# hzykent/LiDAL

Hardware: AMD Instinct MI355X
Metric: voxels/sec SPVCNN fwd+bwd @120k pts (higher is better)
Workload: dtype bf16; 1 GPU; spvcnn train step (train.py:127-140: fwd + CE + bwd + Adam), 5 scans x ~120k pts per GPU, 0.05 m voxels, kernel maps rebuilt every step (each step builds the next step's coordinate tables on a second stream; variants.inline_geometry: built inside the forward pass); parallelism=dp1

## Files before the change

include/lidal_amd.h:

```cpp
#ifndef LIDAL_AMD_H
#define LIDAL_AMD_H

#include <stdint.h>

#ifdef __cplusplus
extern "C" {
#endif

#define LIDAL_F32 0
#define LIDAL_BF16 1
#define LIDAL_F32_SPLIT 2

const char* lidal_last_error(void);
int lidal_version(void);

int lidal_hash(const int32_t* coords, int64_t n, int64_t* out, void* stream);
int lidal_floor_coords(const float* coords, int64_t n, int stride, int32_t* out, void* stream);
int lidal_revoxelize_coords(const float* coords, int64_t n, float init_res, float after_res, float* out_float,
                            int32_t* out_floor, void* stream);
int lidal_kernel_hash(const int32_t* coords, int64_t n, const int32_t* offsets, int k,
                      int64_t* out, void* stream);

int64_t lidal_hash_table_bytes(int64_t n_keys);
int lidal_hash_table_build(const int64_t* keys, int64_t n, void* table, int64_t table_bytes,
// ... 141 lines not shown
int lidal_conv_wgrad_streams(const void* a, const void* b, int64_t n_a, int64_t n_b, const int32_t* spairs,
                             const int32_t* sdesc, int n_wg, int a_col, float* gw, float* partial, int64_t n_slabs,
                             int k, int ca, int cb, int dtype, void* stream);

int64_t lidal_bn_workspace_bytes(int64_t n, int c);
int lidal_bn_train_fwd(const void* x, int dtype, int64_t n, int c, const float* gamma,
                       const float* beta, float eps, float momentum, float* running_mean,
                       float* running_var, int64_t* num_batches_tracked, int relu,
                       const void* residual, void* y, float* save_mean, float* save_invstd, void* ws,
                       int64_t ws_bytes, void* stream);
int lidal_bn_train_fwd_tiles(const void* x, int dtype, int64_t n, int c, const float* gamma,
                             const float* beta, float eps, float momentum, float* running_mean,
                             float* running_var, int64_t* num_batches_tracked, int relu,
                             const void* residual, void* y, float* save_mean, float* save_invstd,
                             const float* tile_stats, int64_t n_tiles, void* stream);
int lidal_bn_eval_fwd(const void* x, int dtype, int64_t n, int c, const float* gamma,
                      const float* beta, const float* running_mean, const float* running_var,
                      float eps, int relu, void* y, void* stream);
int lidal_bn_bwd(const void* x, const void* dy, int64_t dy_stride, int dtype, int64_t n, int c, const float* gamma,
                 const float* beta, int relu, const float* save_mean, const float* save_invstd,
                 void* dx, float* grad_gamma, float* grad_beta, void* ws, int64_t ws_bytes,
                 void* stream);
int lidal_bn_bwd_tiles(const void* x, const void* dy, int64_t dy_stride, int dtype, int64_t n, int c,
                       const float* gamma, const float* beta, int relu, const float* save_mean,
                       const float* save_invstd, void* dx, float* grad_gamma, float* grad_beta,
                       const float* tile_sums, int64_t n_tiles, void* stream);
int lidal_add_relu_bwd_bn_sums(const void* out, const void* g, void* gm, int dtype, int64_t n, int c,
                               const void* x_a, const float* mean_a, const float* invstd_a, void* part_a,
                               const void* x_b, const float* mean_b, const float* invstd_b, void* part_b,
                               int64_t part_bytes, void* stream);
// ... 132 lines not shown

enum {
  LIDAL_OP_CONV_WEIGHT_IMAGE_BATCH = 1, LIDAL_OP_CONV_APPLY_IMAGE = 2, LIDAL_OP_CONV_DGRAD_BN_SUMS = 3,
  LIDAL_OP_CONV_WGRAD = 4, LIDAL_OP_BN_TRAIN_FWD = 5, LIDAL_OP_BN_TRAIN_FWD_TILES = 6, LIDAL_OP_BN_BWD = 7,
  LIDAL_OP_BN_BWD_TILES = 8, LIDAL_OP_BN_EVAL_FWD = 9, LIDAL_OP_BN_FOLD = 10, LIDAL_OP_COLSUM = 11,
  LIDAL_OP_ADD_RELU_FWD = 12, LIDAL_OP_ADD_RELU_BWD = 13, LIDAL_OP_VOXELIZE_FWD_1TO1 = 14,
  LIDAL_OP_VOXELIZE_FWD_SORTED = 15, LIDAL_OP_VOXELIZE_BWD = 16, LIDAL_OP_DEVOXELIZE_FWD = 17,
  LIDAL_OP_DEVOXELIZE_BWD_SORTED = 18, LIDAL_OP_CE_FWD = 19, LIDAL_OP_CE_BWD = 20, LIDAL_OP_COPY2D = 21,
  LIDAL_OP_ADD2D = 22, LIDAL_OP_TRANSPOSE_F32 = 23, LIDAL_OP_CAST_ROWS_BF16 = 24, LIDAL_OP_VIEW_MEAN_SOFTMAX = 25,
  LIDAL_OP_FORK_SIDE = 26, LIDAL_OP_JOIN_SIDE = 27, LIDAL_OP_CONV_APPLY_IMAGE_WS = 28,
  LIDAL_OP_CONV_DGRAD_BN_SUMS_WS = 29, LIDAL_OP_ADD_RELU_BWD_BN_SUMS = 30, LIDAL_OP_BN_BWD_FROM_SUMS = 31,
  LIDAL_OP_ADD_RELU_BWD_BN_TILE_SUMS = 32, LIDAL_OP_DEVOXELIZE_BWD_CELLS = 33,
  LIDAL_OP_CONV_WGRAD_STREAMS = 34
};
#define LIDAL_OP_FLAG_SIDE 1
int lidal_plan_op_args(int kind);
int lidal_debug_read(const void* dev, void* host, int64_t nbytes);
int lidal_plan_run(const int64_t* words, int64_t n_words, int64_t n_ops, void* stream, void* side_stream);
int lidal_plan_run_streams(const int64_t* words, int64_t n_words, int64_t n_ops, void* const* streams, int n_streams);

#ifdef __cplusplus
}
#endif
#endif
```

lidal_amd/backend.py:

```python
import ctypes
import os

import torch

_HERE = os.path.dirname(os.path.abspath(__file__))
LIB_PATH = os.environ.get('LIDAL_AMD_LIB') or os.path.join(_HERE, 'liblidal_amd.so')

F32, BF16 = 0, 1
_lib = None
HITS = {}


def hit(name):
    HITS[name] = HITS.get(name, 0) + 1

_vp, _i32, _i64, _f32, _f64 = (ctypes.c_void_p, ctypes.c_int, ctypes.c_int64, ctypes.c_float,
                               ctypes.c_double)

SIGNATURES = {
    'lidal_last_error': (ctypes.c_char_p, []),
    'lidal_version': (_i32, []),
    'lidal_floor_coords': (_i32, [_vp, _i64, _i32, _vp, _vp]),
    'lidal_revoxelize_coords': (_i32, [_vp, _i64, _f32, _f32, _vp, _vp, _vp]),
    'lidal_hash': (_i32, [_vp, _i64, _vp, _vp]),
# ... 63 lines not shown
                                           _vp, _vp, _vp, _vp, _i32, _vp, _vp, _i64, _vp]),
    'lidal_conv_wgrad_slabs': (_i64, [_i64, _i64, _i32, _i32, _i32, _i32]),
    'lidal_conv_wgrad': (_i32, [_vp, _vp, _i64, _i64, _vp, _vp, _i32, _vp, _vp, _i64, _i32, _i32, _i32, _i32, _vp]),
    'lidal_conv_wgrad_streams': (_i32, [_vp, _vp, _i64, _i64, _vp, _vp, _i32, _i32, _vp, _vp, _i64, _i32, _i32, _i32, _i32, _vp]),
    'lidal_conv_wgrad_streams_serves': (_i32, [_i64, _i64, _i32, _i32, _i32]),
    'lidal_wgrad_streams_workgroups': (_i32, []),
    'lidal_wgrad_streams_rules': (_i64, [_i64, _i32, _i32]),
    'lidal_wgrad_streams_desc_words': (_i64, [_i32, _i32]),
    'lidal_wgrad_streams_workspace_bytes': (_i64, [_i64, _i32]),
    'lidal_wgrad_streams_build': (_i32, [_vp, _vp, _i32, _i64, _vp, _i32, _i64, _i32, _vp, _i64, _vp, _vp, _i64, _vp]),
    'lidal_bn_workspace_bytes': (_i64, [_i64, _i32]),
    'lidal_bn_train_fwd': (_i32, [_vp, _i32, _i64, _i32, _vp, _vp, _f32, _f32, _vp, _vp, _vp, _i32, _vp, _vp, _vp,
                                  _vp, _vp, _i64, _vp]),
    'lidal_bn_train_fwd_tiles': (_i32, [_vp, _i32, _i64, _i32, _vp, _vp, _f32, _f32, _vp, _vp, _vp, _i32, _vp, _vp,
                                        _vp, _vp, _vp, _i64, _vp]),
    'lidal_bn_eval_fwd': (_i32, [_vp, _i32, _i64, _i32, _vp, _vp, _vp, _vp, _f32, _i32, _vp, _vp]),
    'lidal_bn_bwd': (_i32, [_vp, _vp, _i64, _i32, _i64, _i32, _vp, _vp, _i32, _vp, _vp, _vp, _vp, _vp, _vp,
                            _i64, _vp]),
    'lidal_bn_bwd_tiles': (_i32, [_vp, _vp, _i64, _i32, _i64, _i32, _vp, _vp, _i32, _vp, _vp, _vp, _vp, _vp, _vp,
                                  _i64, _vp]),
    'lidal_add_relu_bwd_bn_sums': (_i32, [_vp, _vp, _vp, _i32, _i64, _i32, _vp, _vp, _vp, _vp, _vp, _vp, _vp, _vp, _i64, _vp]),
    'lidal_add_relu_bwd_bn_tile_sums': (_i32, [_vp, _vp, _vp, _i32, _i64, _i32, _vp, _vp, _vp, _vp, _vp, _vp, _vp, _vp, _i64, _vp]),
    'lidal_bn_tail_parts': (_i64, [_i64, _i32, _i32]),
    'lidal_bn_bwd_from_sums': (_i32, [_vp, _vp, _i64, _i32, _i64, _i32, _vp, _vp, _i32, _vp, _vp, _vp, _vp, _vp, _vp,
                                      _i64, _vp]),
    'lidal_bn_set_fused': (_i32, [_i32]),
    'lidal_bn_set_slab_sums': (_i32, [_i32]),
    'lidal_bn_check_device': (_i32, []),
    'lidal_bn_fold': (_i32, [_vp, _vp, _vp, _vp, _f32, _i32, _vp, _vp, _vp]),
    'lidal_colsum': (_i32, [_vp, _i32, _i64, _i32, _vp, _vp, _i64, _vp]),
# ... 433 lines not shown
```

lidal_amd/csrc/bn.hip:

```cpp
#include "common.h"
#include <type_traits>

using namespace lidal;

namespace {

constexpr int NT = 256;
constexpr int EW_THREADS = 256;
constexpr int UNR = 4;
constexpr int UNR_S = UNR, UNR_A = UNR, UNR_P = UNR, UNR_D = UNR;
constexpr int MIN_ROWS_PER_WG = 32;

template <typename T> struct IO;
template <> struct IO<float> {
  static constexpr int VEC = 4;
  typedef float4 vec;
  __device__ static void unpack(const vec& v, float (&f)[4]) { f[0] = v.x; f[1] = v.y; f[2] = v.z; f[3] = v.w; }
  __device__ static vec pack(const float (&f)[4]) { return make_float4(f[0], f[1], f[2], f[3]); }
};
typedef __attribute__((ext_vector_type(8))) __bf16 bf16x8_t;
template <> struct IO<__bf16> {
  static constexpr int VEC = 8;
  typedef bf16x8_t vec;
  __device__ static void unpack(const vec& v, float (&f)[8]) {
// ... 143 lines not shown
    if (running_mean != nullptr) {
      const float unbiased = (float)(na > 1. ? qa / (na - 1.) : var);
      running_mean[ch] = (1.f - momentum) * running_mean[ch] + momentum * (float)ma;
      running_var[ch] = (1.f - momentum) * running_var[ch] + momentum * unbiased;
    }
  }
}

template <typename T, bool VAR_IN>
__global__ void __launch_bounds__(NT) bn_apply_kernel(const T* __restrict__ x, int64_t n, int c,
                                                      const float* __restrict__ mean,
                                                      const float* __restrict__ istd_or_var,
                                                      const float* __restrict__ gamma,
                                                      const float* __restrict__ beta, float eps,
                                                      int relu, const T* __restrict__ res,
                                                      T* __restrict__ y, int rpw) {
  constexpr int VEC = IO<T>::VEC;
  const int cg_n = c / VEC, rpi = NT / cg_n;
  const int tid = threadIdx.x, cg = tid % cg_n, rl = tid / cg_n;
  if (rl >= rpi) return;
  const int64_t r_beg = (int64_t)blockIdx.x * rpw;
  const int64_t r_end = (r_beg + rpw < n) ? r_beg + rpw : n;
  float mu[VEC], sc[VEC], sh[VEC], iv[VEC];
  load_channels<VEC>(mean, cg * VEC, 0.f, mu);
  load_channels<VEC>(istd_or_var, cg * VEC, 0.f, iv);
  load_channels<VEC>(gamma, cg * VEC, 1.f, sc);
  load_channels<VEC>(beta, cg * VEC, 0.f, sh);
#pragma unroll
  for (int i = 0; i < VEC; ++i) {
    const float is = VAR_IN ? 1.f / sqrtf(iv[i] + eps) : iv[i];
    sc[i] = is * sc[i];
// ... 2 lines not shown
  constexpr int F = decltype(fc)::value;
  constexpr bool RELU1 = (F & 1) != 0, HAS_RES = (F & 2) != 0, RELU2 = (F & 4) != 0;
  auto one = [&](const typename IO<T>::vec& v, const typename IO<T>::vec& vr, int64_t r) {
    float f[VEC], fr[VEC];
    IO<T>::unpack(v, f);
    if (HAS_RES) IO<T>::unpack(vr, fr);
#pragma unroll
    for (int i = 0; i < VEC; ++i) {
      f[i] = (f[i] - mu[i]) * sc[i] + sh[i];
      if (RELU1) f[i] = fmaxf(f[i], 0.f);
      if (HAS_RES) {
        f[i] = (float)(T)f[i] + fr[i];
        if (RELU2) f[i] = fmaxf(f[i], 0.f);
      }
    }
    *reinterpret_cast<typename IO<T>::vec*>(y + r * c + cg * VEC) = IO<T>::pack(f);
  };
  const T* rsrc = HAS_RES ? res : x;
  int64_t r = r_beg + rl;
  for (; r + (UNR_A - 1) * rpi < r_end; r += UNR_A * rpi) {
    typename IO<T>::vec v[UNR_A], vr[UNR_A];
#pragma unroll
    for (int u = 0; u < UNR_A; ++u)
      v[u] = *reinterpret_cast<const typename IO<T>::vec*>(x + (r + u * rpi) * c + cg * VEC);
    if (HAS_RES) {
#pragma unroll
      for (int u = 0; u < UNR_A; ++u)
        vr[u] = *reinterpret_cast<const typename IO<T>::vec*>(rsrc + (r + u * rpi) * c + cg * VEC);
    } else {
#pragma unroll
      for (int u = 0; u < UNR_A; ++u) vr[u] = v[u];
// ... 437 lines not shown
static inline int rows_per_wg(int64_t n) { return slab_rows(n); }
constexpr int64_t EW_WIDE_BYTES = 12ll << 20;
static inline int rows_per_wg_ew(int64_t n, int64_t row_bytes) {
  const int wgs = n * row_bytes >= EW_WIDE_BYTES ? 2 * BN_WGS : BN_WGS;
  int64_t rpw = (n + wgs - 1) / wgs;
  if (rpw < MIN_ROWS_PER_WG) rpw = MIN_ROWS_PER_WG;
  return (int)rpw;
}
static inline int nslabs_ew(int64_t n, int64_t row_bytes) {
  return (int)cdiv(n > 0 ? n : 1, rows_per_wg_ew(n, row_bytes));
}
static inline int nparts_for(int64_t n) { return (int)cdiv(n > 0 ? n : 1, rows_per_wg(n)); }
template <typename T>
int bn_train_fwd(const void* x, int64_t n, int c, const float* gamma, const float* beta, float eps,
                 float momentum, float* rm, float* rv, long long* nbt, int relu, const void* res,
                 void* y, float* mean, float* invstd, double* part, hipStream_t s) {
  constexpr int VEC = IO<T>::VEC;
  int np = nparts_for(n);
  bn_stats_partial_kernel<T><<<np, NT, 2 * NT * VEC * sizeof(double), s>>>((const T*)x, n, c, part,
                                                                           rows_per_wg(n));
  LIDAL_CHECK_LAUNCH("bn_stats_partial");
  bn_stats_final_kernel<double><<<(unsigned)cdiv(c, 8), NT, 0, s>>>(part, np, c, eps, momentum, mean,
                                                             invstd, rm, rv, nbt);
  LIDAL_CHECK_LAUNCH("bn_stats_final");
  bn_apply_kernel<T, false><<<nslabs_ew(n, (int64_t)c * sizeof(T)), NT, 0, s>>>((const T*)x, n, c, mean, invstd, gamma,
                                                        beta, eps, relu, (const T*)res, (T*)y,
                                                        rows_per_wg_ew(n, (int64_t)c * sizeof(T)));
  LIDAL_CHECK_LAUNCH("bn_apply");
  return 0;
}

template <typename T, bool TILES>
bool bn_bwd_merge_dx(const void* x, const void* dy, int64_t ldy, int64_t n, int c, const float* gamma, const float* beta,
                     int relu, const float* mean, const float* invstd, void* dx, float* ggamma, float* gbeta,
                     const void* part, int nparts, hipStream_t s);

static int g_slab_sums = -1;
static inline bool slab_sums_enabled() {
  if (g_slab_sums < 0) { const char* e = getenv("LIDAL_BN_SLAB_SUMS"); g_slab_sums = (e && e[0] == '0') ? 0 : 1; }
  return g_slab_sums != 0;
}
__global__ void __launch_bounds__(NT) bn_bwd_tiles_final_kernel(const float* __restrict__ part, int nparts, int c,
// ... 120 lines not shown
extern "C" int lidal_bn_check_device(void);
static int bn_check(int64_t n, int c, int dtype) {
  if (int rc = lidal_bn_check_device()) return rc;
  int vec = dtype == LIDAL_BF16 ? 8 : 4;
  LIDAL_REQUIRE(dtype == LIDAL_F32 || dtype == LIDAL_BF16, "bn: bad dtype %d", dtype);
  LIDAL_REQUIRE(c > 0 && c % vec == 0 && c / vec <= NT, "bn: channels %d must be a multiple of %d and <= %d",
                c, vec, NT * vec);
  LIDAL_REQUIRE(n >= 0, "bn: bad row count");
  return 0;
}

extern "C" int64_t lidal_bn_workspace_bytes(int64_t n, int c) {
  return (int64_t)nparts_for(n) * c * 3 * sizeof(double) + 256;
}

extern "C" int lidal_bn_train_fwd(const void* x, int dtype, int64_t n, int c, const float* gamma,
                                  const float* beta, float eps, float momentum,
                                  float* running_mean, float* running_var,
                                  int64_t* num_batches_tracked, int relu, const void* residual,
                                  void* y, float* save_mean, float* save_invstd, void* ws,
                                  int64_t ws_bytes, void* stream) {
  if (int rc = bn_check(n, c, dtype)) return rc;
  LIDAL_REQUIRE(n > 0, "bn_train_fwd: needs at least one row");
  LIDAL_REQUIRE(ws_bytes >= lidal_bn_workspace_bytes(n, c), "bn workspace too small");
  hipStream_t s = (hipStream_t)stream;
  if (dtype == LIDAL_F32)
    return bn_train_fwd<float>(x, n, c, gamma, beta, eps, momentum, running_mean, running_var,
                               (long long*)num_batches_tracked, relu, residual, y, save_mean,
                               save_invstd, (double*)ws, s);
  return bn_train_fwd<__bf16>(x, n, c, gamma, beta, eps, momentum, running_mean, running_var,
                              (long long*)num_batches_tracked, relu, residual, y, save_mean,
                              save_invstd, (double*)ws, s);
}

__global__ void __launch_bounds__(NT) bn_tiles_final_kernel(const float* __restrict__ part, int nparts,
                                                            int c, float eps, float momentum,
                                                            float* __restrict__ mean,
                                                            float* __restrict__ invstd,
                                                            float* __restrict__ running_mean,
                                                            float* __restrict__ running_var,
                                                            long long* __restrict__ num_batches) {
  __shared__ double sn[NT], s1[NT], s2[NT];
  const int tid = threadIdx.x, ch = blockIdx.x;
  if (num_batches != nullptr && ch == 0 && tid == 0) *num_batches += 1;
  double n = 0., a = 0., b = 0.;
  for (int p = tid; p < nparts; p += NT) {
    const float* s = part + ((int64_t)ch * nparts + p) * 3;
// ... 41 lines not shown
    __builtin_amdgcn_s_sleep(2);
    v = __hip_atomic_load(s.v + idx, __ATOMIC_RELAXED, __HIP_MEMORY_SCOPE_AGENT);
  }
  return __uint_as_float((unsigned)v);
}

template <typename T, int NTT, int F>
__global__ void __launch_bounds__(NTT) bn_apply_tiles_kernel(const T* __restrict__ x, int64_t n, int c,
                                                            const float* __restrict__ part, int nparts, float eps,
                                                            float momentum, float* __restrict__ mean,
                                                            float* __restrict__ invstd, float* __restrict__ running_mean,
                                                            float* __restrict__ running_var,
                                                            long long* __restrict__ num_batches,
                                                            const float* __restrict__ gamma, const float* __restrict__ beta,
                                                            const T* __restrict__ res, T* __restrict__ y, int rpw,
                                                            Slots slots) {
  constexpr bool RELU1 = (F & 1) != 0, HAS_RES = (F & 2) != 0, RELU2 = (F & 4) != 0;
  constexpr int VEC = IO<T>::VEC;
  __shared__ double sn[NTT], s1[NTT], s2[NTT];
  __shared__ float smu[SLOT_CH], sis[SLOT_CH];
  const int tid = threadIdx.x;
  if (num_batches != nullptr && blockIdx.x == 0 && tid == 0) *num_batches += 1;
  for (int ch = blockIdx.x; ch < c; ch += gridDim.x) {
    double nn = 0., a = 0., b = 0.;
    for (int p0 = tid; tid < NT && p0 < nparts; p0 += 8 * NT) {
      float t0[8], t1[8], t2[8];
#pragma unroll
      for (int u = 0; u < 8; ++u) {
        const int p = p0 + u * NT;
        const float* sp = part + ((int64_t)ch * nparts + (p < nparts ? p : p0)) * 3;
        t0[u] = sp[0]; t1[u] = sp[1]; t2[u] = sp[2];
// ... 62 lines not shown
    sc[i] = sis[ch] * sc[i];
  }
  auto one = [&](const typename IO<T>::vec& v, const typename IO<T>::vec& vr, int64_t r) {
    float f[VEC], fr[VEC];
    IO<T>::unpack(v, f);
    if (HAS_RES) IO<T>::unpack(vr, fr);
#pragma unroll
    for (int i = 0; i < VEC; ++i) {
      f[i] = (f[i] - mu[i]) * sc[i] + sh[i];
      if (RELU1) f[i] = fmaxf(f[i], 0.f);
      if (HAS_RES) {
        f[i] = (float)(T)f[i] + fr[i];
        if (RELU2) f[i] = fmaxf(f[i], 0.f);
      }
    }
    *reinterpret_cast<typename IO<T>::vec*>(y + r * c + cg * VEC) = IO<T>::pack(f);
  };
  if (first) {
#pragma unroll
    for (int u = 0; u < UNR_A; ++u) one(v0[u], HAS_RES ? vr0[u] : v0[u], r + u * rpi);
    r += UNR_A * rpi;
  }
  for (; r + (UNR_A - 1) * rpi < r_end; r += UNR_A * rpi) {
    typename IO<T>::vec v[UNR_A], vr[UNR_A];
#pragma unroll
    for (int u = 0; u < UNR_A; ++u)
      v[u] = *reinterpret_cast<const typename IO<T>::vec*>(x + (r + u * rpi) * c + cg * VEC);
    if (HAS_RES) {
#pragma unroll
      for (int u = 0; u < UNR_A; ++u)
        vr[u] = *reinterpret_cast<const typename IO<T>::vec*>(rsrc + (r + u * rpi) * c + cg * VEC);
// ... 233 lines not shown
                     const void* part, int nparts, hipStream_t s) {
  Slots slots;
  if (dx == nullptr || !bn_fused() || c > SLOT_CH || !next_slots(&slots, s)) return false;
  if (relu)
    bn_bwd_dx_merge_kernel<T, TILES, true><<<nslabs_ew(n, (int64_t)c * sizeof(T)), NT, 0, s>>>(
        (const T*)x, (const T*)dy, n, c, mean, invstd, gamma, beta, relu, part, nparts, gbeta, ggamma, (T*)dx,
        rows_per_wg_ew(n, (int64_t)c * sizeof(T)), ldy, slots);
  else
    bn_bwd_dx_merge_kernel<T, TILES, false><<<nslabs_ew(n, (int64_t)c * sizeof(T)), NT, 0, s>>>(
        (const T*)x, (const T*)dy, n, c, mean, invstd, gamma, beta, relu, part, nparts, gbeta, ggamma, (T*)dx,
        rows_per_wg_ew(n, (int64_t)c * sizeof(T)), ldy, slots);
  return true;
}
}

extern "C" int lidal_bn_train_fwd_tiles(const void* x, int dtype, int64_t n, int c, const float* gamma,
                                        const float* beta, float eps, float momentum,
                                        float* running_mean, float* running_var,
                                        int64_t* num_batches_tracked, int relu,
                                        const void* residual, void* y, float* save_mean,
                                        float* save_invstd, const float* tile_stats, int64_t n_tiles,
                                        void* stream) {
  if (int rc = bn_check(n, c, dtype)) return rc;
  LIDAL_REQUIRE(n > 0 && n_tiles > 0 && tile_stats != nullptr, "bn_train_fwd_tiles: needs rows and tile statistics");
  hipStream_t s = (hipStream_t)stream;
  Slots slots;
  if (bn_fused() && c <= SLOT_CH && next_slots(&slots, s)) {
    const int flags = (relu & 1) | (residual != nullptr ? 2 : 0) | ((residual != nullptr && (relu & 2)) ? 4 : 0);
#define LIDAL_APPLY_TILES(T, FV)                                                                                          \
    bn_apply_tiles_kernel<T, EW_THREADS, FV><<<nslabs_ew(n, (int64_t)c * sizeof(T)), EW_THREADS, 0, s>>>(                 \
        (const T*)x, n, c, tile_stats, (int)n_tiles, eps, momentum, save_mean, save_invstd, running_mean, running_var,    \
        (long long*)num_batches_tracked, gamma, beta, (const T*)residual, (T*)y, rows_per_wg_ew(n, (int64_t)c * sizeof(T)), \
        slots)
#define LIDAL_APPLY_TILES_F(T)                                                        \
    switch (flags) {                                                                  \
      case 0: LIDAL_APPLY_TILES(T, 0); break; case 1: LIDAL_APPLY_TILES(T, 1); break; \
      case 2: LIDAL_APPLY_TILES(T, 2); break; case 3: LIDAL_APPLY_TILES(T, 3); break; \
      case 6: LIDAL_APPLY_TILES(T, 6); break; default: LIDAL_APPLY_TILES(T, 7); break; \
    }
    if (dtype == LIDAL_F32) { LIDAL_APPLY_TILES_F(float) } else { LIDAL_APPLY_TILES_F(__bf16) }
#undef LIDAL_APPLY_TILES_F
#undef LIDAL_APPLY_TILES
    LIDAL_CHECK_LAUNCH("bn_apply(tiles merged in the launch)");
    return 0;
  }
  bn_tiles_final_kernel<<<(unsigned)c, NT, 0, s>>>(tile_stats, (int)n_tiles, c, eps, momentum, save_mean,
                                                   save_invstd, running_mean, running_var,
                                                   (long long*)num_batches_tracked);
  LIDAL_CHECK_LAUNCH("bn_stats_final(tiles)");
  if (dtype == LIDAL_F32)
    bn_apply_kernel<float, false><<<nslabs_ew(n, (int64_t)c * 4), NT, 0, s>>>((const float*)x, n, c, save_mean, save_invstd,
                                                              gamma, beta, eps, relu,
                                                              (const float*)residual, (float*)y,
                                                              rows_per_wg_ew(n, (int64_t)c * 4));
  else
    bn_apply_kernel<__bf16, false><<<nslabs_ew(n, (int64_t)c * 2), NT, 0, s>>>((const __bf16*)x, n, c, save_mean,
                                                               save_invstd, gamma, beta, eps, relu,
                                                               (const __bf16*)residual, (__bf16*)y,
                                                               rows_per_wg_ew(n, (int64_t)c * 2));
  LIDAL_CHECK_LAUNCH("bn_apply");
  return 0;
}

extern "C" int lidal_bn_eval_fwd(const void* x, int dtype, int64_t n, int c, const float* gamma,
                                 const float* beta, const float* running_mean,
                                 const float* running_var, float eps, int relu, void* y,
                                 void* stream) {
  if (int rc = bn_check(n, c, dtype)) return rc;
  if (n == 0) return 0;
  hipStream_t s = (hipStream_t)stream;
  if (dtype == LIDAL_F32)
    bn_apply_kernel<float, true><<<nslabs_ew(n, (int64_t)c * 4), NT, 0, s>>>(
        (const float*)x, n, c, running_mean, running_var, gamma, beta, eps, relu, nullptr, (float*)y,
        rows_per_wg_ew(n, (int64_t)c * 4));
  else
    bn_apply_kernel<__bf16, true><<<nslabs_ew(n, (int64_t)c * 2), NT, 0, s>>>(
        (const __bf16*)x, n, c, running_mean, running_var, gamma, beta, eps, relu, nullptr, (__bf16*)y,
        rows_per_wg_ew(n, (int64_t)c * 2));
  LIDAL_CHECK_LAUNCH("lidal_bn_eval_fwd");
  return 0;
}

extern "C" int lidal_bn_bwd(const void* x, const void* dy, int64_t dy_stride, int dtype, int64_t n, int c,
                            const float* gamma, const float* beta, int relu,
                            const float* save_mean, const float* save_invstd, void* dx,
                            float* grad_gamma, float* grad_beta, void* ws, int64_t ws_bytes,
                            void* stream) {
  if (int rc = bn_check(n, c, dtype)) return rc;
  LIDAL_REQUIRE(n > 0, "bn_bwd: needs at least one row");
  LIDAL_REQUIRE(ws_bytes >= lidal_bn_workspace_bytes(n, c), "bn workspace too small");
  const int vec = dtype == LIDAL_F32 ? 4 : 8;
  LIDAL_REQUIRE(dy_stride >= c && dy_stride % vec == 0, "bn_bwd: dy row stride %lld (rows of %d, 16-byte steps)",
                (long long)dy_stride, c);
// ... 184 lines not shown
```

lidal_amd/csrc/error.cpp:

```cpp
#include <stdarg.h>
#include <stdio.h>

#include "../../include/lidal_amd.h"

namespace lidal {
static thread_local char g_err[512] = "";
void set_error(const char* fmt, ...) {
  va_list ap;
  va_start(ap, fmt);
  vsnprintf(g_err, sizeof(g_err), fmt, ap);
  va_end(ap);
}
}

extern "C" const char* lidal_last_error(void) { return lidal::g_err; }
extern "C" int lidal_version(void) { return 165; }
```

lidal_amd/csrc/plan.hip:

```cpp
#include <string.h>
#include <mutex>

#include "common.h"

using namespace lidal;

namespace {

typedef __attribute__((ext_vector_type(8))) __bf16 bf16x8_t;

template <typename U>
__global__ void __launch_bounds__(256) copy2d_kernel(const U* __restrict__ src, int64_t src_pitch,
                                                     U* __restrict__ dst, int64_t dst_pitch, int64_t rows,
                                                     int row_units, int zero_units) {
  const int per = row_units + zero_units;
  const int64_t total = rows * per;
  const int64_t stride = (int64_t)gridDim.x * 256;
  for (int64_t i = (int64_t)blockIdx.x * 256 + threadIdx.x; i < total; i += stride) {
    const int64_t r = i / per;
    const int u = (int)(i - r * per);
    U v;
    if (u < row_units) v = src[r * src_pitch + u];
    else memset(&v, 0, sizeof(U));
    dst[r * dst_pitch + u] = v;
// ... 288 lines not shown
        break;
      case LIDAL_OP_CONV_DGRAD_BN_SUMS_WS:
        rc = lidal_conv_dgrad_bn_sums_ws(P(0), P(1), CP(int32_t, 2), CP(int32_t, 3), CP(uint32_t, 4), P(5), L(6), L(7),
                                         I(8), I(9), I(10), I(11), I(12), P(13), CP(float, 14), CP(float, 15),
                                         CP(float, 16), CP(float, 17), I(18), MP(float, 19), P(20), L(21), st);
        break;
      case LIDAL_OP_CONV_WGRAD:
        rc = lidal_conv_wgrad(P(0), P(1), L(2), L(3), CP(int32_t, 4), CP(int64_t, 5), I(6), MP(float, 7), MP(float, 8),
                              L(9), I(10), I(11), I(12), I(13), st);
        break;
      case LIDAL_OP_CONV_WGRAD_STREAMS:
        rc = lidal_conv_wgrad_streams(P(0), P(1), L(2), L(3), CP(int32_t, 4), CP(int32_t, 5), I(6), I(7), MP(float, 8),
                                      MP(float, 9), L(10), I(11), I(12), I(13), I(14), st);
        break;
      case LIDAL_OP_BN_TRAIN_FWD:
        rc = lidal_bn_train_fwd(P(0), I(1), L(2), I(3), CP(float, 4), CP(float, 5), F(6), F(7), MP(float, 8),
                                MP(float, 9), MP(int64_t, 10), I(11), P(12), P(13), MP(float, 14), MP(float, 15), P(16),
                                L(17), st);
        break;
      case LIDAL_OP_BN_TRAIN_FWD_TILES:
        rc = lidal_bn_train_fwd_tiles(P(0), I(1), L(2), I(3), CP(float, 4), CP(float, 5), F(6), F(7), MP(float, 8),
                                      MP(float, 9), MP(int64_t, 10), I(11), P(12), P(13), MP(float, 14), MP(float, 15),
                                      CP(float, 16), L(17), st);
        break;
      case LIDAL_OP_BN_BWD:
        rc = lidal_bn_bwd(P(0), P(1), L(2), I(3), L(4), I(5), CP(float, 6), CP(float, 7), I(8), CP(float, 9),
                          CP(float, 10), P(11), MP(float, 12), MP(float, 13), P(14), L(15), st);
        break;
      case LIDAL_OP_BN_BWD_FROM_SUMS:
        rc = lidal_bn_bwd_from_sums(P(0), P(1), L(2), I(3), L(4), I(5), CP(float, 6), CP(float, 7), I(8), CP(float, 9),
                                    CP(float, 10), P(11), MP(float, 12), MP(float, 13), P(14), L(15), st);
        break;
      case LIDAL_OP_ADD_RELU_BWD_BN_SUMS:
        rc = lidal_add_relu_bwd_bn_sums(P(0), P(1), P(2), I(3), L(4), I(5), P(6), CP(float, 7), CP(float, 8), P(9), P(10),
                                        CP(float, 11), CP(float, 12), P(13), L(14), st);
        break;
      case LIDAL_OP_ADD_RELU_BWD_BN_TILE_SUMS:
        rc = lidal_add_relu_bwd_bn_tile_sums(P(0), P(1), P(2), I(3), L(4), I(5), P(6), CP(float, 7), CP(float, 8),
                                             MP(float, 9), P(10), CP(float, 11), CP(float, 12), MP(float, 13), L(14), st);
// ... 103 lines not shown
```

lidal_amd/network/plan.py:

```python
import array
import ctypes
import os
import struct

import torch

from .. import backend as B
from ..nn.functional import conv as _C
from ..nn.functional import norm as _N
from ..nn.functional import devoxelize as _DV
from ..nn.functional.invlist import inverse_lists
from ..nn.functional.voxelize import _index32

__all__ = ['planned_forward', 'enabled', 'COUNTERS']

ENABLED = os.environ.get('LIDAL_PLAN', '1') != '0'
BN_SUMS = None

OP_CONV_WEIGHT_IMAGE_BATCH, OP_CONV_APPLY_IMAGE, OP_CONV_DGRAD_BN_SUMS, OP_CONV_WGRAD = 1, 2, 3, 4
OP_BN_TRAIN_FWD, OP_BN_TRAIN_FWD_TILES, OP_BN_BWD, OP_BN_BWD_TILES, OP_BN_EVAL_FWD, OP_BN_FOLD = 5, 6, 7, 8, 9, 10
OP_COLSUM, OP_ADD_RELU_FWD, OP_ADD_RELU_BWD, OP_VOXELIZE_FWD_1TO1, OP_VOXELIZE_FWD_SORTED = 11, 12, 13, 14, 15
OP_VOXELIZE_BWD, OP_DEVOXELIZE_FWD, OP_DEVOXELIZE_BWD_SORTED, OP_CE_FWD, OP_CE_BWD = 16, 17, 18, 19, 20
OP_COPY2D, OP_ADD2D, OP_TRANSPOSE_F32, OP_CAST_ROWS_BF16, OP_VIEW_MEAN_SOFTMAX = 21, 22, 23, 24, 25
OP_FORK_SIDE, OP_JOIN_SIDE, OP_CONV_APPLY_IMAGE_WS, OP_CONV_DGRAD_BN_SUMS_WS = 26, 27, 28, 29
OP_ADD_RELU_BWD_BN_SUMS, OP_BN_BWD_FROM_SUMS, OP_ADD_RELU_BWD_BN_TILE_SUMS, OP_DEVOXELIZE_BWD_CELLS = 30, 31, 32, 33
OP_CONV_WGRAD_STREAMS = 34

COUNTERS = {'ops': 0, 'plans': 0}
TALLY = os.environ.get('LIDAL_PLAN_TALLY', '0') != '0'
TRACE = None
SIDE_ROWS = int(os.environ.get('LIDAL_PLAN_SIDE_ROWS', str(1 << 40)))
SIDE_F32 = os.environ.get('LIDAL_PLAN_SIDE_F32', '0') == '1'
BRANCH_ROWS = int(os.environ.get('LIDAL_PLAN_BRANCH_ROWS', '100000'))
POINT_SIDE = int(os.environ.get('LIDAL_PLAN_POINT_SIDE', '1'))
F32_BN_ALONE = os.environ.get('LIDAL_PLAN_F32_BN_ALONE', '1') != '0'
_NARGS = {}
_HIT_NAMES = {1: 'conv_weight_image', 2: 'conv_apply', 3: 'conv_apply', 4: 'conv_wgrad', 5: 'bn_train_fwd',
              6: 'bn_train_fwd', 7: 'bn_bwd', 8: 'bn_bwd', 9: 'bn_eval_fwd', 10: 'bn_fold', 11: 'colsum',
              12: 'add_relu_fwd', 13: 'add_relu_bwd', 14: 'voxelize_fwd_1to1', 15: 'voxelize_fwd_sorted',
              16: 'voxelize_bwd', 17: 'devoxelize_fwd', 18: 'devoxelize_bwd_sorted', 19: 'ce_fwd', 20: 'ce_bwd',
              21: 'copy2d', 22: 'add2d', 23: 'transpose_f32', 24: 'cast_rows_bf16', 25: 'view_mean_softmax',
# ... 595 lines not shown
        wb = _C.apply_workspace_bytes(n_out, c.co)
        self.w += (OP_CONV_APPLY_IMAGE_WS, x, c.img_f, table[0], table[1], table[2], out, n_in, n_out, ci, c.co, c.k, 0,
                   self.ccode(c), 0, 0, 0, 0, st, self.scratch(wb) if wb else 0, wb)
        self.nops += 1
        return out, st

    def f_dense(self, c, x, n, co, shift, stats, flag=0):
        A = self.arena
        out = A.alloc(n * co * self.esz)
        st = A.alloc(-(-n // self.tile) * co * 12) if (stats and self.bf16) else 0
        self.w += (OP_CONV_APPLY_IMAGE | flag, x, c.img_f, 0, 0, 0, out, n, n, c.ci, co, 1, 0, self.ccode(c),
                   self.ones if shift else 0, shift, 0, 0, st)
        self.nops += 1
        return out, st

    def f_bn(self, r, x, n, st, residual=0, relu_after=False, flag=0):
        A, p = self.arena, self.ptr
        c = r.c
        y = A.alloc(n * c * self.esz)
        mean = A.alloc(c * 4)
        invstd = A.alloc(c * 4)
        relu = r.relu | (2 if (relu_after and residual) else 0)
        if st:
            self.w += (OP_BN_TRAIN_FWD_TILES | flag, x, self.code, n, c, p[r.w], p[r.b], r.eps, r.mom, p[r.rm], p[r.rv],
                       p[r.nbt], relu, residual, y, mean, invstd, st, -(-n // self.tile))
        else:
            nb = _bn_ws(n, c)
            self.w += (OP_BN_TRAIN_FWD | flag, x, self.code, n, c, p[r.w], p[r.b], r.eps, r.mom, p[r.rm], p[r.rv],
                       p[r.nbt], relu, residual, y, mean, invstd, self.scratch(nb, flag), nb)
        self.nops += 1
        return y, mean, invstd

    def f_conv_bn(self, cb, x, n_in, table, n_out, ci=None):
        c, r = cb
        x1, st = self.f_conv(c, x, n_in, c.ci if ci is None else ci, table, n_out, True)
        y, mean, invstd = self.f_bn(r, x1, n_out, st)
        self.saved[id(cb)] = (x, x1, mean, invstd)
        return y

    def f_res(self, r, x, n, table):
        fl = 0
        if r.cs is not None:
            fl = self.fork(2) if (BRANCH_ROWS and n >= BRANCH_ROWS) else 0
            xs, sts = self.f_dense(r.cs, x, n, r.cs.co, 0, True, fl)
            res, means, invs = self.f_bn(r.bs, xs, n, sts, flag=fl)
        else:
            xs = means = invs = 0
            res = x
        x1, st1 = self.f_conv(r.c1, x, n, r.c1.ci, table, n, True)
        y1, mean1, inv1 = self.f_bn(r.b1, x1, n, st1)
        x2, st2 = self.f_conv(r.c2, y1, n, r.c2.ci, table, n, True)
        if fl:
            self.join(2)
        out, mean2, inv2 = self.f_bn(r.b2, x2, n, st2, res, True)
        self.saved[id(r)] = (x, x1, mean1, inv1, y1, x2, mean2, inv2, out, xs, means, invs)
        return out

    def f_cat(self, a, ca, b, cb, n):
        A, e = self.arena, self.esz
        out = A.alloc(n * (ca + cb) * e)
        pitch = (ca + cb) * e
        self.w += (OP_COPY2D, a, ca * e, out, pitch, n, ca * e, 0,
                   OP_COPY2D, b, cb * e, out + ca * e, pitch, n, cb * e, 0)
        self.nops += 2
        return out

    def f_devox(self, x, lvl, c):
        t = self.T.pt[lvl]
        P = self.T.p
# ... 59 lines not shown
        prog, T, A = self.prog, self.T, self.arena
        n = T.n
        k3, k2 = T.k3, T.k2
        bf = self.bf16
        x = self.feats.data_ptr()
        if prog.spvcnn:
            x = self.f_vox(x, 0, 4, B.F32)
        c0 = prog.stem[0][0]
        if bf:
            xc = A.alloc(n[0] * 8 * 2)
            self.w += (OP_CAST_ROWS_BF16, x, 4, xc, 8, n[0])
            self.nops += 1
            x, ci0 = xc, 8
        else:
            ci0 = 4
        y = self.f_conv_bn(prog.stem[0], x, n[0], k3[0], n[0], ci0)
        x0 = self.f_conv_bn(prog.stem[1], y, n[0], k3[0], n[0])
        skips = [x0]
        cs = [c0.co]
        if prog.spvcnn:
            z0 = self.f_devox(x0, 0, cs[0])
            pre = self.f_point_lin(prog.points[0], z0) if self.TRAIN else None
            y = self.f_vox(z0, 0, cs[0])
        else:
            y = x0
        for l, (down, ra, rb) in enumerate(prog.stages):
            y = self.f_conv_bn(down, y, n[l], k2[l][0:3], n[l + 1])
            y = self.f_res(ra, y, n[l + 1], k3[l + 1])
            y = self.f_res(rb, y, n[l + 1], k3[l + 1])
            skips.append(y)
            cs.append(rb.c2.co)
        z = None
        if prog.spvcnn:
            z1 = self.f_point(prog.points[0], z0, self.f_devox(y, 4, cs[4]), pre)
            pre = self.f_point_lin(prog.points[1], z1) if self.TRAIN else None
            y = self.f_vox(z1, 4, cs[4])
            self.f_dropout(y, n[4], cs[4])
            z = z1
        for i, (dec, ra, rb) in enumerate(prog.ups):
            l = 3 - i
            y = self.f_conv_bn(dec, y, n[l + 1], k2[l][3:6], n[l])
            y = self.f_cat(y, dec[0].co, skips[l], cs[l], n[l])
            y = self.f_res(ra, y, n[l], k3[l])
            y = self.f_res(rb, y, n[l], k3[l])
            c_out = rb.c2.co
            if prog.spvcnn and i == 1:
                z2 = self.f_point(prog.points[1], z, self.f_devox(y, 2, c_out), pre)
                pre = self.f_point_lin(prog.points[2], z2) if self.TRAIN else None
                y = self.f_vox(z2, 2, c_out)
                self.f_dropout(y, n[2], c_out)
                z = z2
        if prog.spvcnn:
            feat = self.f_point(prog.points[2], z, self.f_devox(y, 0, c_out), pre)
            rows = T.p
        else:
            feat, rows = y, n[0]
        logits, co_pad = self.f_classifier(feat, rows)
# ... 431 lines not shown
```

Before: 29.36 million voxels/s.

## Fuse skip concatenation into BN apply via pitched dual-output writes

```diff
diff --git a/include/lidal_amd.h b/include/lidal_amd.h
--- a/include/lidal_amd.h
+++ b/include/lidal_amd.h
@@ -179,6 +179,17 @@
                              float* running_var, int64_t* num_batches_tracked, int relu,
                              const void* residual, void* y, float* save_mean, float* save_invstd,
                              const float* tile_stats, int64_t n_tiles, void* stream);
+int lidal_bn_train_fwd_pitched(const void* x, int dtype, int64_t n, int c, const float* gamma,
+                               const float* beta, float eps, float momentum, float* running_mean,
+                               float* running_var, int64_t* num_batches_tracked, int relu,
+                               const void* residual, void* y, int64_t y_pitch, void* y2, int64_t y2_pitch,
+                               float* save_mean, float* save_invstd, void* ws, int64_t ws_bytes, void* stream);
+int lidal_bn_train_fwd_tiles_pitched(const void* x, int dtype, int64_t n, int c, const float* gamma,
+                                     const float* beta, float eps, float momentum, float* running_mean,
+                                     float* running_var, int64_t* num_batches_tracked, int relu,
+                                     const void* residual, void* y, int64_t y_pitch, void* y2, int64_t y2_pitch,
+                                     float* save_mean, float* save_invstd, const float* tile_stats,
+                                     int64_t n_tiles, void* stream);
 int lidal_bn_eval_fwd(const void* x, int dtype, int64_t n, int c, const float* gamma,
                       const float* beta, const float* running_mean, const float* running_var,
                       float eps, int relu, void* y, void* stream);
@@ -341,6 +352,7 @@
   LIDAL_OP_CONV_WGRAD_STREAMS = 34
 };
 #define LIDAL_OP_FLAG_SIDE 1
+#define LIDAL_OP_FLAG_WITH_COPY 16
 int lidal_plan_op_args(int kind);
 int lidal_debug_read(const void* dev, void* host, int64_t nbytes);
 int lidal_plan_run(const int64_t* words, int64_t n_words, int64_t n_ops, void* stream, void* side_stream);
diff --git a/lidal_amd/backend.py b/lidal_amd/backend.py
--- a/lidal_amd/backend.py
+++ b/lidal_amd/backend.py
@@ -101,6 +101,10 @@
                                   _vp, _vp, _i64, _vp]),
     'lidal_bn_train_fwd_tiles': (_i32, [_vp, _i32, _i64, _i32, _vp, _vp, _f32, _f32, _vp, _vp, _vp, _i32, _vp, _vp,
                                         _vp, _vp, _vp, _i64, _vp]),
+    'lidal_bn_train_fwd_pitched': (_i32, [_vp, _i32, _i64, _i32, _vp, _vp, _f32, _f32, _vp, _vp, _vp, _i32, _vp, _vp,
+                                          _i64, _vp, _i64, _vp, _vp, _vp, _i64, _vp]),
+    'lidal_bn_train_fwd_tiles_pitched': (_i32, [_vp, _i32, _i64, _i32, _vp, _vp, _f32, _f32, _vp, _vp, _vp, _i32, _vp,
+                                                _vp, _i64, _vp, _i64, _vp, _vp, _vp, _i64, _vp]),
     'lidal_bn_eval_fwd': (_i32, [_vp, _i32, _i64, _i32, _vp, _vp, _vp, _vp, _f32, _i32, _vp, _vp]),
     'lidal_bn_bwd': (_i32, [_vp, _vp, _i64, _i32, _i64, _i32, _vp, _vp, _i32, _vp, _vp, _vp, _vp, _vp, _vp,
                             _i64, _vp]),
diff --git a/lidal_amd/csrc/bn.hip b/lidal_amd/csrc/bn.hip
--- a/lidal_amd/csrc/bn.hip
+++ b/lidal_amd/csrc/bn.hip
@@ -181,7 +181,8 @@
                                                       const float* __restrict__ gamma,
                                                       const float* __restrict__ beta, float eps,
                                                       int relu, const T* __restrict__ res,
-                                                      T* __restrict__ y, int rpw) {
+                                                      T* __restrict__ y, int rpw, int64_t ldy,
+                                                      T* __restrict__ y2, int64_t ldy2) {
   constexpr int VEC = IO<T>::VEC;
   const int cg_n = c / VEC, rpi = NT / cg_n;
   const int tid = threadIdx.x, cg = tid % cg_n, rl = tid / cg_n;
@@ -214,7 +215,9 @@
         if (RELU2) f[i] = fmaxf(f[i], 0.f);
       }
     }
-    *reinterpret_cast<typename IO<T>::vec*>(y + r * c + cg * VEC) = IO<T>::pack(f);
+    const typename IO<T>::vec o = IO<T>::pack(f);
+    *reinterpret_cast<typename IO<T>::vec*>(y + r * ldy + cg * VEC) = o;
+    if (y2 != nullptr) *reinterpret_cast<typename IO<T>::vec*>(y2 + r * ldy2 + cg * VEC) = o;
   };
   const T* rsrc = HAS_RES ? res : x;
   int64_t r = r_beg + rl;
@@ -682,7 +685,8 @@
 template <typename T>
 int bn_train_fwd(const void* x, int64_t n, int c, const float* gamma, const float* beta, float eps,
                  float momentum, float* rm, float* rv, long long* nbt, int relu, const void* res,
-                 void* y, float* mean, float* invstd, double* part, hipStream_t s) {
+                 void* y, int64_t ldy, void* y2, int64_t ldy2, float* mean, float* invstd, double* part,
+                 hipStream_t s) {
   constexpr int VEC = IO<T>::VEC;
   int np = nparts_for(n);
   bn_stats_partial_kernel<T><<<np, NT, 2 * NT * VEC * sizeof(double), s>>>((const T*)x, n, c, part,
@@ -693,7 +697,8 @@
   LIDAL_CHECK_LAUNCH("bn_stats_final");
   bn_apply_kernel<T, false><<<nslabs_ew(n, (int64_t)c * sizeof(T)), NT, 0, s>>>((const T*)x, n, c, mean, invstd, gamma,
                                                         beta, eps, relu, (const T*)res, (T*)y,
-                                                        rows_per_wg_ew(n, (int64_t)c * sizeof(T)));
+                                                        rows_per_wg_ew(n, (int64_t)c * sizeof(T)), ldy, (T*)y2,
+                                                        ldy2);
   LIDAL_CHECK_LAUNCH("bn_apply");
   return 0;
 }
@@ -844,6 +849,39 @@
   return (int64_t)nparts_for(n) * c * 3 * sizeof(double) + 256;
 }
 
+static int bn_pitch_check(const char* who, int c, int dtype, const void* y, int64_t y_pitch) {
+  const int64_t row = (int64_t)c * (dtype == LIDAL_BF16 ? 2 : 4);
+  LIDAL_REQUIRE(((uintptr_t)y & 15) == 0, "%s: output must be 16-byte aligned", who);
+  LIDAL_REQUIRE(y_pitch >= row, "%s: output pitch %lld bytes is below the row length %lld", who, (long long)y_pitch,
+                (long long)row);
+  LIDAL_REQUIRE(y_pitch % 16 == 0, "%s: output pitch %lld bytes is not a multiple of 16", who, (long long)y_pitch);
+  LIDAL_REQUIRE(y_pitch < (1ll << 24), "%s: output pitch %lld bytes must be below 2^24", who, (long long)y_pitch);
+  return 0;
+}
+
+extern "C" int lidal_bn_train_fwd_pitched(const void* x, int dtype, int64_t n, int c, const float* gamma,
+                                          const float* beta, float eps, float momentum,
+                                          float* running_mean, float* running_var,
+                                          int64_t* num_batches_tracked, int relu, const void* residual,
+                                          void* y, int64_t y_pitch, void* y2, int64_t y2_pitch, float* save_mean,
+                                          float* save_invstd, void* ws, int64_t ws_bytes, void* stream) {
+  LIDAL_REQUIRE(dtype == LIDAL_F32 || dtype == LIDAL_BF16, "bn: bad dtype %d", dtype);
+  if (int rc = bn_pitch_check("bn_train_fwd", c, dtype, y, y_pitch)) return rc;
+  if (y2 != nullptr)
+    if (int rc = bn_pitch_check("bn_train_fwd (second output)", c, dtype, y2, y2_pitch)) return rc;
+  if (int rc = bn_check(n, c, dtype)) return rc;
+  LIDAL_REQUIRE(n > 0, "bn_train_fwd: needs at least one row");
+  LIDAL_REQUIRE(ws_bytes >= lidal_bn_workspace_bytes(n, c), "bn workspace too small");
+  hipStream_t s = (hipStream_t)stream;
+  if (dtype == LIDAL_F32)
+    return bn_train_fwd<float>(x, n, c, gamma, beta, eps, momentum, running_mean, running_var,
+                               (long long*)num_batches_tracked, relu, residual, y, y_pitch / 4, y2, y2_pitch / 4,
+                               save_mean, save_invstd, (double*)ws, s);
+  return bn_train_fwd<__bf16>(x, n, c, gamma, beta, eps, momentum, running_mean, running_var,
+                              (long long*)num_batches_tracked, relu, residual, y, y_pitch / 2, y2, y2_pitch / 2,
+                              save_mean, save_invstd, (double*)ws, s);
+}
+
 extern "C" int lidal_bn_train_fwd(const void* x, int dtype, int64_t n, int c, const float* gamma,
                                   const float* beta, float eps, float momentum,
                                   float* running_mean, float* running_var,
@@ -851,16 +889,9 @@
                                   void* y, float* save_mean, float* save_invstd, void* ws,
                                   int64_t ws_bytes, void* stream) {
   if (int rc = bn_check(n, c, dtype)) return rc;
-  LIDAL_REQUIRE(n > 0, "bn_train_fwd: needs at least one row");
-  LIDAL_REQUIRE(ws_bytes >= lidal_bn_workspace_bytes(n, c), "bn workspace too small");
-  hipStream_t s = (hipStream_t)stream;
-  if (dtype == LIDAL_F32)
-    return bn_train_fwd<float>(x, n, c, gamma, beta, eps, momentum, running_mean, running_var,
-                               (long long*)num_batches_tracked, relu, residual, y, save_mean,
-                               save_invstd, (double*)ws, s);
-  return bn_train_fwd<__bf16>(x, n, c, gamma, beta, eps, momentum, running_mean, running_var,
-                              (long long*)num_batches_tracked, relu, residual, y, save_mean,
-                              save_invstd, (double*)ws, s);
+  return lidal_bn_train_fwd_pitched(x, dtype, n, c, gamma, beta, eps, momentum, running_mean, running_var,
+                                    num_batches_tracked, relu, residual, y, (int64_t)c * (dtype == LIDAL_BF16 ? 2 : 4),
+                                    nullptr, 0, save_mean, save_invstd, ws, ws_bytes, stream);
 }
 
 __global__ void __launch_bounds__(NT) bn_tiles_final_kernel(const float* __restrict__ part, int nparts,
@@ -932,7 +963,7 @@
                                                             long long* __restrict__ num_batches,
                                                             const float* __restrict__ gamma, const float* __restrict__ beta,
                                                             const T* __restrict__ res, T* __restrict__ y, int rpw,
-                                                            Slots slots) {
+                                                            int64_t ldy, T* __restrict__ y2, int64_t ldy2, Slots slots) {
   constexpr bool RELU1 = (F & 1) != 0, HAS_RES = (F & 2) != 0, RELU2 = (F & 4) != 0;
   constexpr int VEC = IO<T>::VEC;
   __shared__ double sn[NTT], s1[NTT], s2[NTT];
@@ -1025,7 +1056,9 @@
         if (RELU2) f[i] = fmaxf(f[i], 0.f);
       }
     }
-    *reinterpret_cast<typename IO<T>::vec*>(y + r * c + cg * VEC) = IO<T>::pack(f);
+    const typename IO<T>::vec o = IO<T>::pack(f);
+    *reinterpret_cast<typename IO<T>::vec*>(y + r * ldy + cg * VEC) = o;
+    if (y2 != nullptr) *reinterpret_cast<typename IO<T>::vec*>(y2 + r * ldy2 + cg * VEC) = o;
   };
   if (first) {
 #pragma unroll
@@ -1289,14 +1322,19 @@
 }
 }
 
-extern "C" int lidal_bn_train_fwd_tiles(const void* x, int dtype, int64_t n, int c, const float* gamma,
-                                        const float* beta, float eps, float momentum,
-                                        float* running_mean, float* running_var,
-                                        int64_t* num_batches_tracked, int relu,
-                                        const void* residual, void* y, float* save_mean,
-                                        float* save_invstd, const float* tile_stats, int64_t n_tiles,
-                                        void* stream) {
+extern "C" int lidal_bn_train_fwd_tiles_pitched(const void* x, int dtype, int64_t n, int c, const float* gamma,
+                                                const float* beta, float eps, float momentum,
+                                                float* running_mean, float* running_var,
+                                                int64_t* num_batches_tracked, int relu,
+                                                const void* residual, void* y, int64_t y_pitch, void* y2,
+                                                int64_t y2_pitch, float* save_mean, float* save_invstd,
+                                                const float* tile_stats, int64_t n_tiles, void* stream) {
+  LIDAL_REQUIRE(dtype == LIDAL_F32 || dtype == LIDAL_BF16, "bn: bad dtype %d", dtype);
+  if (int rc = bn_pitch_check("bn_train_fwd_tiles", c, dtype, y, y_pitch)) return rc;
+  if (y2 != nullptr)
+    if (int rc = bn_pitch_check("bn_train_fwd_tiles (second output)", c, dtype, y2, y2_pitch)) return rc;
   if (int rc = bn_check(n, c, dtype)) return rc;
+  const int64_t ldy = y_pitch / (dtype == LIDAL_BF16 ? 2 : 4), ldy2 = y2_pitch / (dtype == LIDAL_BF16 ? 2 : 4);
   LIDAL_REQUIRE(n > 0 && n_tiles > 0 && tile_stats != nullptr, "bn_train_fwd_tiles: needs rows and tile statistics");
   hipStream_t s = (hipStream_t)stream;
   Slots slots;
@@ -1306,7 +1344,7 @@
     bn_apply_tiles_kernel<T, EW_THREADS, FV><<<nslabs_ew(n, (int64_t)c * sizeof(T)), EW_THREADS, 0, s>>>(                 \
         (const T*)x, n, c, tile_stats, (int)n_tiles, eps, momentum, save_mean, save_invstd, running_mean, running_var,    \
         (long long*)num_batches_tracked, gamma, beta, (const T*)residual, (T*)y, rows_per_wg_ew(n, (int64_t)c * sizeof(T)), \
-        slots)
+        ldy, (T*)y2, ldy2, slots)
 #define LIDAL_APPLY_TILES_F(T)                                                        \
     switch (flags) {                                                                  \
       case 0: LIDAL_APPLY_TILES(T, 0); break; case 1: LIDAL_APPLY_TILES(T, 1); break; \
@@ -1327,14 +1365,28 @@
     bn_apply_kernel<float, false><<<nslabs_ew(n, (int64_t)c * 4), NT, 0, s>>>((const float*)x, n, c, save_mean, save_invstd,
                                                               gamma, beta, eps, relu,
                                                               (const float*)residual, (float*)y,
-                                                              rows_per_wg_ew(n, (int64_t)c * 4));
+                                                              rows_per_wg_ew(n, (int64_t)c * 4), ldy, (float*)y2, ldy2);
   else
     bn_apply_kernel<__bf16, false><<<nslabs_ew(n, (int64_t)c * 2), NT, 0, s>>>((const __bf16*)x, n, c, save_mean,
                                                                save_invstd, gamma, beta, eps, relu,
                                                                (const __bf16*)residual, (__bf16*)y,
-                                                               rows_per_wg_ew(n, (int64_t)c * 2));
+                                                               rows_per_wg_ew(n, (int64_t)c * 2), ldy, (__bf16*)y2, ldy2);
   LIDAL_CHECK_LAUNCH("bn_apply");
   return 0;
+}
+
+extern "C" int lidal_bn_train_fwd_tiles(const void* x, int dtype, int64_t n, int c, const float* gamma,
+                                        const float* beta, float eps, float momentum,
+                                        float* running_mean, float* running_var,
+                                        int64_t* num_batches_tracked, int relu,
+                                        const void* residual, void* y, float* save_mean,
+                                        float* save_invstd, const float* tile_stats, int64_t n_tiles,
+                                        void* stream) {
+  if (int rc = bn_check(n, c, dtype)) return rc;
+  return lidal_bn_train_fwd_tiles_pitched(x, dtype, n, c, gamma, beta, eps, momentum, running_mean, running_var,
+                                          num_batches_tracked, relu, residual, y,
+                                          (int64_t)c * (dtype == LIDAL_BF16 ? 2 : 4), nullptr, 0, save_mean, save_invstd,
+                                          tile_stats, n_tiles, stream);
 }
 
 extern "C" int lidal_bn_eval_fwd(const void* x, int dtype, int64_t n, int c, const float* gamma,
@@ -1347,11 +1399,11 @@
   if (dtype == LIDAL_F32)
     bn_apply_kernel<float, true><<<nslabs_ew(n, (int64_t)c * 4), NT, 0, s>>>(
         (const float*)x, n, c, running_mean, running_var, gamma, beta, eps, relu, nullptr, (float*)y,
-        rows_per_wg_ew(n, (int64_t)c * 4));
+        rows_per_wg_ew(n, (int64_t)c * 4), c, nullptr, 0);
   else
     bn_apply_kernel<__bf16, true><<<nslabs_ew(n, (int64_t)c * 2), NT, 0, s>>>(
         (const __bf16*)x, n, c, running_mean, running_var, gamma, beta, eps, relu, nullptr, (__bf16*)y,
-        rows_per_wg_ew(n, (int64_t)c * 2));
+        rows_per_wg_ew(n, (int64_t)c * 2), c, nullptr, 0);
   LIDAL_CHECK_LAUNCH("lidal_bn_eval_fwd");
   return 0;
 }
diff --git a/lidal_amd/csrc/error.cpp b/lidal_amd/csrc/error.cpp
--- a/lidal_amd/csrc/error.cpp
+++ b/lidal_amd/csrc/error.cpp
@@ -14,4 +14,4 @@
 }
 
 extern "C" const char* lidal_last_error(void) { return lidal::g_err; }
-extern "C" int lidal_version(void) { return 165; }
+extern "C" int lidal_version(void) { return 166; }
diff --git a/lidal_amd/csrc/plan.hip b/lidal_amd/csrc/plan.hip
--- a/lidal_amd/csrc/plan.hip
+++ b/lidal_amd/csrc/plan.hip
@@ -326,15 +326,34 @@
                                       MP(float, 9), L(10), I(11), I(12), I(13), I(14), st);
         break;
       case LIDAL_OP_BN_TRAIN_FWD:
-        rc = lidal_bn_train_fwd(P(0), I(1), L(2), I(3), CP(float, 4), CP(float, 5), F(6), F(7), MP(float, 8),
-                                MP(float, 9), MP(int64_t, 10), I(11), P(12), P(13), MP(float, 14), MP(float, 15), P(16),
-                                L(17), st);
-        break;
-      case LIDAL_OP_BN_TRAIN_FWD_TILES:
-        rc = lidal_bn_train_fwd_tiles(P(0), I(1), L(2), I(3), CP(float, 4), CP(float, 5), F(6), F(7), MP(float, 8),
-                                      MP(float, 9), MP(int64_t, 10), I(11), P(12), P(13), MP(float, 14), MP(float, 15),
-                                      CP(float, 16), L(17), st);
-        break;
+      case LIDAL_OP_BN_TRAIN_FWD_TILES: {
+        void* y2 = nullptr;
+        int64_t y2_pitch = 0;
+        const int64_t row = L(3) * (I(1) == LIDAL_BF16 ? 2 : 4);
+        if (flags & LIDAL_OP_FLAG_WITH_COPY) {
+          const int nc = kOps[LIDAL_OP_COPY2D].n_args;
+          LIDAL_REQUIRE(op + 1 < n_ops && pos + 1 + nc <= n_words && (words[pos] & 0xFFFF) == LIDAL_OP_COPY2D
+                        && ((words[pos] >> 16) & 0xFFFF) == sidx, "plan_run: op %lld (%s) is flagged as carrying the copy "
+                        "that follows it, and no copy2d on its stream follows", (long long)op, kOps[kind].name);
+          const int64_t* b = words + pos + 1;
+          LIDAL_REQUIRE(b[0] == a[13] && b[1] == row && b[4] == L(2) && b[5] == row && b[6] == 0 && b[3] >= row,
+                        "plan_run: op %lld (%s): the copy2d that follows is not a copy of this layer's %lld rows of %lld "
+                        "bytes", (long long)op, kOps[kind].name, (long long)L(2), (long long)row);
+          y2 = (void*)(uintptr_t)b[2];
+          y2_pitch = b[3];
+          pos += 1 + nc;
+          ++op;
+        }
+        if (kind == LIDAL_OP_BN_TRAIN_FWD)
+          rc = lidal_bn_train_fwd_pitched(P(0), I(1), L(2), I(3), CP(float, 4), CP(float, 5), F(6), F(7), MP(float, 8),
+                                          MP(float, 9), MP(int64_t, 10), I(11), P(12), P(13), row, y2, y2_pitch,
+                                          MP(float, 14), MP(float, 15), P(16), L(17), st);
+        else
+          rc = lidal_bn_train_fwd_tiles_pitched(P(0), I(1), L(2), I(3), CP(float, 4), CP(float, 5), F(6), F(7),
+                                                MP(float, 8), MP(float, 9), MP(int64_t, 10), I(11), P(12), P(13), row, y2,
+                                                y2_pitch, MP(float, 14), MP(float, 15), CP(float, 16), L(17), st);
+        break;
+      }
       case LIDAL_OP_BN_BWD:
         rc = lidal_bn_bwd(P(0), P(1), L(2), I(3), L(4), I(5), CP(float, 6), CP(float, 7), I(8), CP(float, 9),
                           CP(float, 10), P(11), MP(float, 12), MP(float, 13), P(14), L(15), st);
diff --git a/lidal_amd/network/plan.py b/lidal_amd/network/plan.py
--- a/lidal_amd/network/plan.py
+++ b/lidal_amd/network/plan.py
@@ -25,6 +25,7 @@
 OP_FORK_SIDE, OP_JOIN_SIDE, OP_CONV_APPLY_IMAGE_WS, OP_CONV_DGRAD_BN_SUMS_WS = 26, 27, 28, 29
 OP_ADD_RELU_BWD_BN_SUMS, OP_BN_BWD_FROM_SUMS, OP_ADD_RELU_BWD_BN_TILE_SUMS, OP_DEVOXELIZE_BWD_CELLS = 30, 31, 32, 33
 OP_CONV_WGRAD_STREAMS = 34
+FLAG_WITH_COPY = 16 << 16
 
 COUNTERS = {'ops': 0, 'plans': 0}
 TALLY = os.environ.get('LIDAL_PLAN_TALLY', '0') != '0'
@@ -650,31 +651,35 @@
         self.nops += 1
         return out, st
 
-    def f_bn(self, r, x, n, st, residual=0, relu_after=False, flag=0):
+    def f_bn(self, r, x, n, st, residual=0, relu_after=False, flag=0, dup=None):
         A, p = self.arena, self.ptr
         c = r.c
         y = A.alloc(n * c * self.esz)
         mean = A.alloc(c * 4)
         invstd = A.alloc(c * 4)
         relu = r.relu | (2 if (relu_after and residual) else 0)
+        with_copy = FLAG_WITH_COPY if dup is not None else 0
         if st:
-            self.w += (OP_BN_TRAIN_FWD_TILES | flag, x, self.code, n, c, p[r.w], p[r.b], r.eps, r.mom, p[r.rm], p[r.rv],
-                       p[r.nbt], relu, residual, y, mean, invstd, st, -(-n // self.tile))
+            self.w += (OP_BN_TRAIN_FWD_TILES | flag | with_copy, x, self.code, n, c, p[r.w], p[r.b], r.eps, r.mom, p[r.rm],
+                       p[r.rv], p[r.nbt], relu, residual, y, mean, invstd, st, -(-n // self.tile))
         else:
             nb = _bn_ws(n, c)
-            self.w += (OP_BN_TRAIN_FWD | flag, x, self.code, n, c, p[r.w], p[r.b], r.eps, r.mom, p[r.rm], p[r.rv],
-                       p[r.nbt], relu, residual, y, mean, invstd, self.scratch(nb, flag), nb)
-        self.nops += 1
+            self.w += (OP_BN_TRAIN_FWD | flag | with_copy, x, self.code, n, c, p[r.w], p[r.b], r.eps, r.mom, p[r.rm],
+                       p[r.rv], p[r.nbt], relu, residual, y, mean, invstd, self.scratch(nb, flag), nb)
+        self.nops += 1
+        if dup is not None:
+            self.w += (OP_COPY2D | flag, y, c * self.esz, dup[0], dup[1], n, c * self.esz, 0)
+            self.nops += 1
         return y, mean, invstd
 
-    def f_conv_bn(self, cb, x, n_in, table, n_out, ci=None):
+    def f_conv_bn(self, cb, x, n_in, table, n_out, ci=None, dup=None):
         c, r = cb
         x1, st = self.f_conv(c, x, n_in, c.ci if ci is None else ci, table, n_out, True)
-        y, mean, invstd = self.f_bn(r, x1, n_out, st)
+        y, mean, invstd = self.f_bn(r, x1, n_out, st, dup=dup)
         self.saved[id(cb)] = (x, x1, mean, invstd)
         return y
 
-    def f_res(self, r, x, n, table):
+    def f_res(self, r, x, n, table, dup=None):
         fl = 0
         if r.cs is not None:
             fl = self.fork(2) if (BRANCH_ROWS and n >= BRANCH_ROWS) else 0
@@ -688,7 +693,7 @@
         x2, st2 = self.f_conv(r.c2, y1, n, r.c2.ci, table, n, True)
         if fl:
             self.join(2)
-        out, mean2, inv2 = self.f_bn(r.b2, x2, n, st2, res, True)
+        out, mean2, inv2 = self.f_bn(r.b2, x2, n, st2, res, True, dup=dup)
         self.saved[id(r)] = (x, x1, mean1, inv1, y1, x2, mean2, inv2, out, xs, means, invs)
         return out
 
@@ -778,8 +783,18 @@
             x, ci0 = xc, 8
         else:
             ci0 = 4
+        e = self.esz
+        cats = {}
+
+        def skip_to(l, c_skip):
+            if not self.TRAIN or l > 3:
+                return {}
+            c_up = prog.ups[3 - l][0][0].co
+            pitch = (c_up + c_skip) * e
+            cats[l] = (A.alloc(n[l] * pitch), pitch)
+            return {'dup': (cats[l][0] + c_up * e, pitch)}
         y = self.f_conv_bn(prog.stem[0], x, n[0], k3[0], n[0], ci0)
-        x0 = self.f_conv_bn(prog.stem[1], y, n[0], k3[0], n[0])
+        x0 = self.f_conv_bn(prog.stem[1], y, n[0], k3[0], n[0], **skip_to(0, c0.co))
         skips = [x0]
         cs = [c0.co]
         if prog.spvcnn:
@@ -791,7 +806,7 @@
         for l, (down, ra, rb) in enumerate(prog.stages):
             y = self.f_conv_bn(down, y, n[l], k2[l][0:3], n[l + 1])
             y = self.f_res(ra, y, n[l + 1], k3[l + 1])
-            y = self.f_res(rb, y, n[l + 1], k3[l + 1])
+            y = self.f_res(rb, y, n[l + 1], k3[l + 1], **skip_to(l + 1, rb.c2.co))
             skips.append(y)
             cs.append(rb.c2.co)
         z = None
@@ -803,8 +818,12 @@
             z = z1
         for i, (dec, ra, rb) in enumerate(prog.ups):
             l = 3 - i
-            y = self.f_conv_bn(dec, y, n[l + 1], k2[l][3:6], n[l])
-            y = self.f_cat(y, dec[0].co, skips[l], cs[l], n[l])
+            if self.TRAIN:
+                self.f_conv_bn(dec, y, n[l + 1], k2[l][3:6], n[l], dup=cats[l])
+                y = cats[l][0]
+            else:
+                y = self.f_conv_bn(dec, y, n[l + 1], k2[l][3:6], n[l])
+                y = self.f_cat(y, dec[0].co, skips[l], cs[l], n[l])
             y = self.f_res(ra, y, n[l], k3[l])
             y = self.f_res(rb, y, n[l], k3[l])
             c_out = rb.c2.co
```

New measurement: 29.56 million voxels/s (median of 6 runs). About the same (+0.7%).
